# Lightbrite88/Argon_Monte_Carlo

Measured on AMD Instinct MI355X. Metric: particle-steps/sec, higher is better.
Workload: dtype f64; 1 GPU; cube_1e5; geometry=cube, n_particles=100000, n_per_gpu=100000, parallelism=single GPU

## Files before the change

argon_monte_carlo_amd/csrc/amc_commit_dev.h:

```cpp
#pragma once
#include "amc_grid_dev.h"

#define AMC_COMMIT_BLOCKS 64

struct amc_commit_args {
    amc_resolve_ctl *ctl;
    const double4 *hist;
    int *ov_head;
    const int *ev_gen;
    const rs_event *ev;
    const int4 *sl_meta;
    const int *sl_hits;
    const uint8_t *sl_moved;
    const double *sl_state;
    int *slot_of;
    int max_slots, max_hist;
    long long lo, hi;
    int count_pp;
    int defer;
    int nogrid;
    int enabled;
    int step;
    const int *od_stall;
    int od_tick;
    int from_wide;
    const int *wctl;
    int *host_ncand;
};

AMC_DEV void amc_commit_part(const amc_commit_args &C, const amc_out &O, const amc_grid &G, const amc_state &S, int gtid,
                             int gstride)
{
    amc_resolve_ctl *ctl = C.ctl;
    int c_active, c_ok, c_nslots, c_nhist, c_ncand, c_nclusters = 0, c_rounds;
    if (C.from_wide) {
        const amc_resolve_ctl *wc = (const amc_resolve_ctl *)C.wctl;
        c_ncand = wc->ncand;
        c_active = c_ncand > 0;
        c_nslots = 2 * c_ncand + wc->nslots; c_nhist = 4 * c_ncand + wc->nhist;
        c_ok = !wc->ovf; c_rounds = 1;
        if (gtid == 0) {
            for (int b = 0; b < 16; b++) c_nclusters += C.wctl[32 + b];
            if (C.host_ncand) *C.host_ncand = c_ncand;
            O.cnt->cand_count = 0;
        }
    } else {
        c_active = ctl->active; c_ok = ctl->ok && !ctl->ovf; c_nslots = ctl->nslots; c_nhist = ctl->nhist;
        c_ncand = ctl->ncand; c_rounds = ctl->rounds;
        if (gtid == 0) c_nclusters = ctl->nclusters;
    }
    if (!c_active) return;
    const bool ok = c_ok != 0;
    const bool defer = ok && C.defer;
    const int ns = c_nslots < C.max_slots ? c_nslots : C.max_slots;
    const int nh = c_nhist < C.max_hist ? c_nhist : C.max_hist;
    int my_hits = 0, my_fp = 0;
    for (int s = gtid; s < ns; s += gstride) {
        const int p = C.sl_meta[s].x;
        if (ok && C.count_pp) { const int hs = C.sl_hits[s]; my_hits += hs & 0xffff; my_fp += hs >> 16; }
        if (defer || p < 0) continue;
        if (ok && C.sl_moved[s]) {
            const double *t = C.sl_state + (size_t)s * RS_SLOT_DOUBLES;
            S.x[p] = t[0]; S.y[p] = t[1]; S.z[p] = t[2]; S.vx[p] = t[3]; S.vy[p] = t[4]; S.vz[p] = t[5];
            S.d[p] = t[6]; S.dx[p] = t[7]; S.dy[p] = t[8]; S.dz[p] = t[9]; S.flag[p] = t[10] != 0.0 ? 1 : 0;
        }
        C.slot_of[p] = -1;
    }
    for (int o = 32; o > 0; o >>= 1) { my_hits += __shfl_down(my_hits, o, 64); my_fp += __shfl_down(my_fp, o, 64); }
    if ((threadIdx.x & 63) == 0 && my_hits) atomicAdd(&O.banks[amc_bank_id()].n_pp, (unsigned long long)my_hits);
    if ((threadIdx.x & 63) == 0 && my_fp) atomicAdd(&O.banks[amc_bank_id()].n_fp_errors, (unsigned long long)my_fp);
    if (ok)
        for (int e = gtid; e < nh; e += gstride) {
            const int g = C.ev_gen[e];
            if (g == 0) continue;
            const rs_event ev = C.ev[e];
            if (g != C.sl_meta[ev.slot].z) continue;
            const int owner = ev.which ? ev.i : ev.j;
            if (owner < C.lo || owner >= C.hi) continue;
            amc_emit(O, ev.phase, ev.cell, ev.i, ev.j, ev.which, ev.val[0], ev.val[1], ev.val[2], ev.val[3]);
        }
    if (!C.nogrid)
        for (int h = gtid; h < nh; h += gstride) {
            const double4 r = C.hist[h];
            int cx, cy, cz;
            amc_grid_coords(G, r.x, r.y, r.z, cx, cy, cz);
            C.ov_head[amc_grid_cell(G, cx, cy, cz, nullptr)] = -1;
        }
    if (gtid == 0) {
        amc_dev_counters *cnt = O.cnt;
        cnt->n_candidates += (unsigned long long)c_ncand;
        cnt->n_clusters += (unsigned long long)c_nclusters;
        cnt->n_rounds += (unsigned long long)c_rounds;
        if (!ok) cnt->flags |= 4ULL;
        ctl->lazy_ns = defer ? ns : 0;
    }
}
```

argon_monte_carlo_amd/csrc/amc_grid.hip:

```cpp
#include <stdlib.h>

#include "amc_grid_dev.h"

#define AMC_CR2_INFLATE (1.0 + 1.0e-9)

__global__ __launch_bounds__(256) void k_bin_lists(const double *__restrict__ x, const double *__restrict__ y,
                                                   const double *__restrict__ z, long long n, amc_grid G, amc_lists B,
                                                   amc_dev_counters *cnt, amc_ovl V)
{
    const long long p = (long long)blockIdx.x * blockDim.x + threadIdx.x;
    if (p >= n) return;
    if (V.skip_epoch && (unsigned int)(V.adj_head[p] >> 32) == V.skip_epoch) return;
    bool outside = false;
    amc_list_insert(G, B, (int)p, x[p], y[p], z[p], &outside);
    if (outside) atomicOr(&cnt->flags, 8ULL);
}

struct amc_adj {
    unsigned long long *head;
    int4 *rec;
    int4 *sd;
    int4 *sl_meta;
    int *sl_hits, *ev_gen;
    unsigned int epoch;
    unsigned long long *mark;
};

AMC_DEV int amc_push_candidate(int a, int b, int max_cand, amc_dev_counters *cnt, const amc_adj &D)
{
    const unsigned int k = atomicAdd(&cnt->cand_count, 1u);
    if (k < (unsigned)max_cand) {
        const int hi = a > b ? a : b, lo = a > b ? b : a;
        int4 r;
        r.x = hi; r.y = lo; r.z = -1; r.w = -1;
        if (D.head) {
            const unsigned long long mine = ((unsigned long long)D.epoch << 32) | (unsigned long long)k;
            const unsigned long long oi = atomicExch(&D.head[hi], mine), oj = atomicExch(&D.head[lo], mine);
            r.z = ((unsigned int)(oi >> 32) == D.epoch) ? (int)(unsigned int)(oi & 0xffffffffULL) : -1;
            r.w = ((unsigned int)(oj >> 32) == D.epoch) ? (int)(unsigned int)(oj & 0xffffffffULL) : -1;
            auto mark = [&](int kd) {
                const unsigned long long old = atomicExch(&D.mark[kd], mine);
                if ((unsigned int)(old >> 32) == D.epoch) D.mark[kd] = ((unsigned long long)D.epoch << 32) | AMC_MARK_MULTI;
            };
            if (r.z >= 0) mark(r.z);
            if (r.w >= 0) mark(r.w);
        }
        D.rec[k] = r;
        D.sd[k] = make_int4(-1, -1, 0, 0);
        if (D.head) {
            D.sl_meta[2 * k] = make_int4(-1, 2 * (int)k, 0, 0);
            D.sl_meta[2 * k + 1] = make_int4(-1, 2 * (int)k + 1, 0, 0);
            atomicAnd(&D.sl_hits[2 * k], 0);
            atomicAnd(&D.sl_hits[2 * k + 1], 0);
            *(int4 *)&D.ev_gen[4 * k] = make_int4(0, 0, 0, 0);
        }
        return (int)k;
    }
    atomicOr(&cnt->flags, 1ULL);
    return -1;
}

AMC_DEV void amc_detect_node(const amc_grid &G, const amc_lists &B, int node, double cr2i, double cr_probe, int max_cand,
                             amc_dev_counters *cnt, const amc_adj &D, const int *od_stall = nullptr, int od_tick = 0)
{
    const int stalled = od_stall ? *od_stall : 0;
    amc_rec me_r = B.rec[node];
    const int live = (B.node_of && node < B.n) ? B.node_of[node] : node;
    if (stalled && od_tick > stalled) return;
    if (me_r.x != me_r.x) {
        if (live == node) return;
        node = live;
        me_r = B.rec[node];
        if (me_r.x != me_r.x) return;
    }
    const int me_p = amc_node_particle(B, node);
    double3 me;
    amc_rec_pos(G, me_r, me.x, me.y, me.z);
    auto found_pair = [&](int q) { amc_push_candidate(me_p, amc_node_particle(B, q), max_cand, cnt, D); };
    int q[9];
    q[0] = amc_rec_next(me_r);
    {
        int ocx, ocy, ocz;
        amc_grid_coords(G, me.x, me.y, me.z, ocx, ocy, ocz);
        const int c_own = amc_grid_cell(G, ocx, ocy, ocz, nullptr);
        int c_lo[4], c_hi[4];
        const int nc = amc_grid_box_ranges(G, me.x, me.y, me.z, cr_probe, c_lo, c_hi);
        int cell[8];
#pragma unroll
        for (int k = 0; k < 4; k++)
#pragma unroll
            for (int t = 0; t < 2; t++) {
                const int c = c_lo[k < nc ? k : 0] + t;
                cell[2 * k + t] = (k < nc && c <= c_hi[k < nc ? k : 0] && c < c_own) ? c : -1;
            }
        unsigned long long hv[8];
#pragma unroll
        for (int e = 0; e < 8; e++) hv[e] = (cell[e] >= 0) ? B.head[cell[e]] : 0ULL;
#pragma unroll
        for (int e = 0; e < 8; e++)
            q[1 + e] = (cell[e] >= 0 && (unsigned int)(hv[e] >> 32) == B.epoch) ? (int)(unsigned int)(hv[e] & 0xffffffffULL) : -1;
    }
    for (;;) {
        bool live = false;
#pragma unroll
        for (int e = 0; e < 9; e++) live |= q[e] >= 0;
        if (!live) break;
        amc_rec o[9];
#pragma unroll
        for (int e = 0; e < 9; e++)
            if (q[e] >= 0) o[e] = B.rec[q[e]];
#pragma unroll
        for (int e = 0; e < 9; e++)
            if (q[e] >= 0) {
                double ox, oy, oz;
                amc_rec_pos(G, o[e], ox, oy, oz);
                const double ex = ox - me.x, ey = oy - me.y, ez = oz - me.z;
                if (ex * ex + ey * ey + ez * ez < cr2i) found_pair(q[e]);
                q[e] = amc_rec_next(o[e]);
            }
    }
}

#ifndef AMC_DETECT_MINW
#define AMC_DETECT_MINW 4
#endif
__global__ __launch_bounds__(256, AMC_DETECT_MINW) void k_detect_lists(amc_grid G, amc_lists B, long long n, double cr2i, double cr_probe,
                                                      int max_cand, amc_dev_counters *cnt, amc_adj D, const int *extra_count,
                                                      int max_extra, const int *od_stall, int od_tick, int *wctl_rearm)
{
    const long long nb = (n + blockDim.x - 1) / blockDim.x;
    if ((long long)blockIdx.x < nb) {
        const long long p = (long long)blockIdx.x * blockDim.x + threadIdx.x;
        if (p < n) amc_detect_node(G, B, (int)p, cr2i, cr_probe, max_cand, cnt, D, od_stall, od_tick);
        if (wctl_rearm && p == 0 && !(*od_stall && od_tick > *od_stall)) {
            amc_resolve_ctl *wc = (amc_resolve_ctl *)wctl_rearm;
            for (int b = 0; b < 16; b++) wctl_rearm[32 + b] = 0;
            wc->nslots = 0; wc->nhist = 0; wc->nedges = 0; wc->nfp = 0; wc->ovf = 0; wc->dirty = 0; wc->nclusters = 0;
            wc->changed = 0; wc->active = 0; wc->cur_round = 1;
        }
        return;
    }
    if (!extra_count) return;
    int ne = *extra_count;
    if (ne > max_extra) ne = max_extra;
    const int stride = (int)((gridDim.x - nb) * blockDim.x);
    for (int e = (int)((blockIdx.x - nb) * blockDim.x + threadIdx.x); e < ne; e += stride)
        amc_detect_node(G, B, (int)n + e, cr2i, cr_probe, max_cand, cnt, D, od_stall, od_tick);
}

__global__ __launch_bounds__(256) void k_detect_own(amc_grid G, amc_lists B, long long lo, long long hi, double cr2i,
                                                    double cr_probe, int *__restrict__ out, int cap, amc_dev_counters *cnt)
{
    const long long p = lo + (long long)blockIdx.x * blockDim.x + threadIdx.x;
    if (p >= hi) return;
    amc_rec me_r = B.rec[p];
    const int live = B.node_of ? B.node_of[p] : (int)p;
    if (me_r.x != me_r.x) {
        if (live == (int)p) return;
        me_r = B.rec[live];
        if (me_r.x != me_r.x) return;
    }
    double3 me;
    amc_rec_pos(G, me_r, me.x, me.y, me.z);
    int c_lo[4], c_hi[4];
    const int nc = amc_grid_box_ranges(G, me.x, me.y, me.z, cr_probe, c_lo, c_hi);
    int q[8];
    unsigned long long hv[8];
#pragma unroll
    for (int k = 0; k < 4; k++)
#pragma unroll
        for (int t = 0; t < 2; t++) {
            const int c = c_lo[k < nc ? k : 0] + t;
            const bool on = k < nc && c <= c_hi[k < nc ? k : 0];
            hv[2 * k + t] = on ? B.head[c] : 0ULL;
            q[2 * k + t] = on ? 0 : -1;
        }
#pragma unroll
    for (int e = 0; e < 8; e++)
        q[e] = (q[e] == 0 && (unsigned int)(hv[e] >> 32) == B.epoch) ? (int)(unsigned int)(hv[e] & 0xffffffffULL) : -1;
    for (;;) {
        bool live = false;
#pragma unroll
        for (int e = 0; e < 8; e++) live |= q[e] >= 0;
        if (!live) break;
        amc_rec o[8];
#pragma unroll
        for (int e = 0; e < 8; e++)
            if (q[e] >= 0) o[e] = B.rec[q[e]];
#pragma unroll
        for (int e = 0; e < 8; e++)
            if (q[e] >= 0) {
                double ox, oy, oz;
                amc_rec_pos(G, o[e], ox, oy, oz);
                const double ex = ox - me.x, ey = oy - me.y, ez = oz - me.z;
                const int pq = amc_node_particle(B, q[e]);
                if (pq < (int)p && ex * ex + ey * ey + ez * ez < cr2i) {
                    const int k = atomicAdd(&out[0], 1);
                    if (k < cap) { out[2 + 2 * k] = (int)p; out[3 + 2 * k] = pq; }
                    else atomicOr(&cnt->flags, 1ULL);
                }
                q[e] = amc_rec_next(o[e]);
            }
    }
}

__global__ __launch_bounds__(256) void k_ingest_candidates(const int *__restrict__ blocks, int world, int block_ints, int cap,
                                                           int max_cand, amc_dev_counters *cnt, amc_adj D, int *__restrict__ own)
{
    const int gtid = blockIdx.x * blockDim.x + threadIdx.x, gstride = gridDim.x * blockDim.x;
    for (int r = 0; r < world; r++) {
        const int *b = blocks + (size_t)r * block_ints;
        int nr = b[0];
        if (nr > cap) {
            nr = cap;
            if (gtid == 0) atomicOr(&cnt->flags, 1ULL);
        }
        for (int k = gtid; k < nr; k += gstride) amc_push_candidate(b[2 + 2 * k], b[3 + 2 * k], max_cand, cnt, D);
    }
    if (gtid == 0) own[0] = 0;
}

#define AP_T 256
__global__ __launch_bounds__(AP_T) void k_detect_allpairs(const double *__restrict__ x, const double *__restrict__ y,
                                                          const double *__restrict__ z, int n, int ntiles, double cr2i,
                                                          int max_cand, amc_dev_counters *cnt, amc_adj D)
{
    int bi = (int)((sqrt(8.0 * (double)blockIdx.x + 1.0) - 1.0) * 0.5);
    while ((long long)(bi + 1) * (bi + 2) / 2 <= (long long)blockIdx.x) bi++;
    while ((long long)bi * (bi + 1) / 2 > (long long)blockIdx.x) bi--;
    const int bj = (int)(blockIdx.x - (long long)bi * (bi + 1) / 2);
    if (bi >= ntiles) return;
    __shared__ double tx[AP_T], ty[AP_T], tz[AP_T];
    const int j0 = bj * AP_T;
    const int jj = j0 + threadIdx.x;
    tx[threadIdx.x] = (jj < n) ? x[jj] : 0.0;
    ty[threadIdx.x] = (jj < n) ? y[jj] : 0.0;
    tz[threadIdx.x] = (jj < n) ? z[jj] : 0.0;
    __syncthreads();
    const int i = bi * AP_T + threadIdx.x;
    if (i >= n) return;
    const double xi = x[i], yi = y[i], zi = z[i];
    int jmax = n - j0;
    if (jmax > AP_T) jmax = AP_T;
    if (bi == bj && jmax > (int)threadIdx.x) jmax = threadIdx.x;
#pragma unroll 4
    for (int k = 0; k < jmax; k++) {
        const double ex = tx[k] - xi, ey = ty[k] - yi, ez = tz[k] - zi;
        const double d2 = fma(ez, ez, fma(ey, ey, ex * ex));
        if (d2 < cr2i) amc_push_candidate(i, j0 + k, max_cand, cnt, D);
    }
}

hipError_t amc_launch_bin(amc_ctx *c)
{
    if (c->allpairs || c->n <= 0) return hipSuccess;
    const long long n = c->n;
    c->B.epoch++;
    c->step.lists_age = -1;
    amc_prof_begin(c, AMC_K_BIN_COUNT);
    amc_ovl V;
    V.adj_head = nullptr; V.skip_epoch = 0;
    AMC_LAUNCH(c, k_bin_lists, dim3((unsigned)((n + 255) / 256)), dim3(256), c->S.x, c->S.y, c->S.z, n,
                       c->G, c->B, c->d_cnt, V);
    amc_prof_end(c);
    return hipGetLastError();
}

hipError_t amc_launch_bin_ovl(amc_ctx *c, int to, unsigned int skip_epoch, hipStream_t stream)
{
    const long long n = c->n;
    amc_ovl V;
    V.adj_head = c->W.adj_head; V.skip_epoch = skip_epoch;
    amc_prof_begin(c, AMC_K_BIN_COUNT);
    AMC_LAUNCH_ON(c, stream, k_bin_lists, dim3((unsigned)((n + 255) / 256)), dim3(256), c->S_buf[to].x, c->S_buf[to].y, c->S_buf[to].z, n,
                  c->G, c->B_buf[to], c->d_cnt, V);
    amc_prof_end(c);
    return hipGetLastError();
}

#define AP2_T 1024
#define AP2_R 4
#define AP2_THREADS (AP2_T / AP2_R)
#define AP2_CHUNK 8
__global__ __launch_bounds__(AP2_THREADS) void k_detect_allpairs_tiled(const double *__restrict__ x, const double *__restrict__ y,
                                                               const double *__restrict__ z, int n, int ntiles, double thr,
                                                               double ox, double oy, double oz,
                                                               int max_cand, amc_dev_counters *cnt, amc_adj D)
{
    int bi = (int)((sqrt(8.0 * (double)blockIdx.x + 1.0) - 1.0) * 0.5);
    while ((long long)(bi + 1) * (bi + 2) / 2 <= (long long)blockIdx.x) bi++;
    while ((long long)bi * (bi + 1) / 2 > (long long)blockIdx.x) bi--;
    const int bj = (int)(blockIdx.x - (long long)bi * (bi + 1) / 2);
    if (bi >= ntiles) return;
    __shared__ double tx[AP2_T], ty[AP2_T], tz[AP2_T], tn[AP2_T];
    const int j0 = bj * AP2_T;
    for (int t = threadIdx.x; t < AP2_T; t += AP2_THREADS) {
        const int jj = j0 + t;
        const bool in = jj < n;
        const double X = in ? x[jj] - ox : 0.0, Y = in ? y[jj] - oy : 0.0, Z = in ? z[jj] - oz : 0.0;
        tx[t] = X; ty[t] = Y; tz[t] = Z;
        tn[t] = in ? fma(Z, Z, fma(Y, Y, X * X)) : 1.0e300;
    }
    __syncthreads();
    int ii[AP2_R];
    double ax[AP2_R], ay[AP2_R], az[AP2_R], ti[AP2_R];
#pragma unroll
    for (int r = 0; r < AP2_R; r++) {
        ii[r] = bi * AP2_T + r * AP2_THREADS + (int)threadIdx.x;
        const bool in = ii[r] < n;
        const double X = in ? x[ii[r]] - ox : 0.0, Y = in ? y[ii[r]] - oy : 0.0, Z = in ? z[ii[r]] - oz : 0.0;
        ax[r] = -2.0 * X; ay[r] = -2.0 * Y; az[r] = -2.0 * Z;
        ti[r] = in ? thr - fma(Z, Z, fma(Y, Y, X * X)) : -1.0e300;
    }
    const bool diag = bi == bj;
    for (int k0 = 0; k0 < AP2_T; k0 += AP2_CHUNK) {
        bool any = false;
#pragma unroll
        for (int u = 0; u < AP2_CHUNK; u++) {
            const double jx = tx[k0 + u], jy = ty[k0 + u], jz = tz[k0 + u], jn = tn[k0 + u];
#pragma unroll
            for (int r = 0; r < AP2_R; r++) any |= fma(az[r], jz, fma(ay[r], jy, fma(ax[r], jx, jn))) < ti[r];
        }
        if (any) {
            for (int u = 0; u < AP2_CHUNK; u++) {
                const int j = j0 + k0 + u;
                const double jx = tx[k0 + u], jy = ty[k0 + u], jz = tz[k0 + u], jn = tn[k0 + u];
#pragma unroll
                for (int r = 0; r < AP2_R; r++)
                    if (fma(az[r], jz, fma(ay[r], jy, fma(ax[r], jx, jn))) < ti[r] && (diag ? j < ii[r] : true))
                        amc_push_candidate(ii[r], j, max_cand, cnt, D);
            }
        }
    }
}

static unsigned int next_sweep_epoch(unsigned int epoch)
{
    epoch = (epoch + 1u) & 0x3fffffffu;
    return epoch ? epoch : 1u;
}

hipError_t amc_launch_detect(amc_ctx *c)
{
    const long long n = c->n;
    if (n <= 0) return hipSuccess;
    const double cr2i = c->allpairs || c->detect_ap ? c->P.collision_range * c->P.collision_range * AMC_CR2_INFLATE : c->G.cr2_probe;
    amc_adj D;
    c->step.sweep_epoch = next_sweep_epoch(c->step.sweep_epoch);
    c->step.plan_split = !c->allpairs && !(c->h_host_ncand && *c->h_host_ncand <= c->plan_small);
    D.head = c->allpairs ? nullptr : c->W.adj_head; D.rec = c->W.cand4; D.sd = c->W.cand_s; D.epoch = c->step.sweep_epoch;
    D.sl_meta = c->W.sl_meta; D.sl_hits = c->W.sl_hits; D.ev_gen = c->W.ev_gen; D.mark = c->W.cand_mark;
    amc_prof_begin(c, AMC_K_DETECT);
    if (c->detect_ap) {
        if (n >= 16 * AP2_T && c->G.ncells > 0) {
            const int ntiles = (int)((n + AP2_T - 1) / AP2_T);
            const long long nblocks = (long long)ntiles * (ntiles + 1) / 2;
            const double ex = c->G.gx * c->G.h, ey = c->G.gy * c->G.h, ez = c->G.gz * c->G.h;
            const double thr = cr2i + 64.0 * 1.1102230246251565e-16 * (ex * ex + ey * ey + ez * ez);
            AMC_LAUNCH(c, k_detect_allpairs_tiled, dim3((unsigned)nblocks), dim3(AP2_THREADS), c->S.x, c->S.y,
                               c->S.z, (int)n, ntiles, thr, c->G.x0, c->G.y0, c->G.z0, c->W.max_cand, c->d_cnt, D);
        } else {
            const int ntiles = (int)((n + AP_T - 1) / AP_T);
            const long long nblocks = (long long)ntiles * (ntiles + 1) / 2;
            if (nblocks > 0)
                AMC_LAUNCH(c, k_detect_allpairs, dim3((unsigned)nblocks), dim3(AP_T), c->S.x, c->S.y,
                                   c->S.z, (int)n, ntiles, cr2i, c->W.max_cand, c->d_cnt, D);
        }
    } else {
        const bool extras = c->B.extra != nullptr && c->keep_K < 2;
        const int slot = (c->B.extra == c->extra_buf[1]) ? 1 : 0;
        const int bs = c->detect_bs;
        AMC_LAUNCH(c, k_detect_lists, dim3((unsigned)((n + bs - 1) / bs) + (extras ? 4u : 0u)), dim3(bs), c->G, c->B, n, cr2i,
                   c->G.cr_probe, c->W.max_cand, c->d_cnt, D, (const int *)(extras ? c->extra_count + slot : nullptr),
                   c->max_extra, (const int *)(c->od_active ? c->d_od : nullptr), c->od_tick,
                   (c->od_active && !c->step.od_prev_ordered) ? c->W.wctl : nullptr);
    }
    amc_prof_end(c);
    return hipGetLastError();
}

hipError_t amc_launch_detect_own(amc_ctx *c)
{
    const long long cnt = c->hi - c->lo;
    amc_prof_begin(c, AMC_K_DETECT);
    if (cnt > 0)
        AMC_LAUNCH(c, k_detect_own, dim3((unsigned)((cnt + 255) / 256)), dim3(256), c->G, c->B, (long long)c->lo, (long long)c->hi,
                   c->G.cr2_probe, c->G.cr_probe, c->MG.cand_send, c->MG.cand_cap, c->d_cnt);
    amc_prof_end(c);
    return hipGetLastError();
}

hipError_t amc_launch_ingest(amc_ctx *c, int world)
{
    amc_adj D;
    c->step.sweep_epoch = next_sweep_epoch(c->step.sweep_epoch);
    c->step.plan_split = !(c->h_host_ncand && *c->h_host_ncand <= c->plan_small);
    D.head = c->W.adj_head; D.rec = c->W.cand4; D.sd = c->W.cand_s; D.epoch = c->step.sweep_epoch;
    D.sl_meta = c->W.sl_meta; D.sl_hits = c->W.sl_hits; D.ev_gen = c->W.ev_gen; D.mark = c->W.cand_mark;
    amc_prof_begin(c, AMC_K_DETECT);
    AMC_LAUNCH(c, k_ingest_candidates, dim3(16), dim3(256), (const int *)c->MG.cand_recv, world, 2 + 2 * c->MG.cand_cap, c->MG.cand_cap,
               c->W.max_cand, c->d_cnt, D, c->MG.cand_send);
    amc_prof_end(c);
    return hipGetLastError();
}
```

argon_monte_carlo_amd/csrc/amc_stream.hip:

```cpp
#include <stdlib.h>
#include <string.h>

#include <algorithm>

#include "amc_commit_dev.h"
#include "amc_energised_dev.h"

struct amc_stream_counts {
    int nwall, nerr, noob, noob_pre;
};

template <int GEOM>
AMC_DEV void amc_stream_particle(amc_particle &q, const amc_params &P, const amc_out &O, double dt, int stages, int ip,
                                 double &px, double &py, double &pz, amc_stream_counts &cn)
{
    if ((stages & AMC_ST_BOUNDS_PRE) && GEOM != AMC_GEOM_CUBE)
        cn.noob_pre = amc_bounds(P, q.x, q.y, q.z, GEOM == AMC_GEOM_PORE_ENERGISED);
    if (stages & AMC_ST_DRIFT) {
        px = q.x; py = q.y; pz = q.z;
        const double sx = dt * q.vx, sy = dt * q.vy, sz = dt * q.vz;
        q.x += sx; q.y += sy; q.z += sz;
        q.d += fabs(sqrt(sx * sx + sy * sy + sz * sz));
        q.dx += fabs(sx); q.dy += fabs(sy); q.dz += fabs(sz);
    }
    if (stages & AMC_ST_WALLS) {
        if (GEOM == AMC_GEOM_CUBE) {
#define AMC_CUBE_AXIS(pos, vel, W)                                                                    \
    if (pos > W) { const double t_ = (pos - W) / vel; vel = -vel; pos = W + t_ * vel; }                \
    if (pos < 0) { const double t_ = pos / vel; vel = -vel; pos = t_ * vel; }
            AMC_CUBE_AXIS(q.x, q.vx, P.cube_x)
            AMC_CUBE_AXIS(q.y, q.vy, P.cube_y)
            AMC_CUBE_AXIS(q.z, q.vz, P.cube_z)
#undef AMC_CUBE_AXIS
        } else if (GEOM == AMC_GEOM_PORE) {
            const double zb = P.z_gap_bottom, zt = P.z_gap_top;
            const double r0 = sqrt(px * px + py * py);
            if (sqrt(q.x * q.x + q.y * q.y) > P.R_oa) {
                if (amc_side_wall(q, P.R_oa_c, true, O, 1, ip)) cn.nerr++; else cn.nwall++;
            }
            if (q.z < 0) { amc_vertical_wall(q, 0.0, O, 2, ip); cn.nwall++; }
            if (q.z > P.H) { amc_vertical_wall(q, P.H, O, 3, ip); cn.nwall++; }
            if ((pz > P.z_cold) && (q.z < P.z_cold) && (sqrt(q.x * q.x + q.y * q.y) > P.R_p)) {
                amc_vertical_wall(q, P.z_cold, O, 4, ip); cn.nwall++;
            }
            if ((pz < P.h_oa) && (q.z > P.h_oa) && (sqrt(q.x * q.x + q.y * q.y) > P.R_p)) {
                amc_vertical_wall(q, P.h_oa, O, 5, ip); cn.nwall++;
            }
            if ((pz < zt) && (pz > zb) && (r0 < P.R_g) && (sqrt(q.x * q.x + q.y * q.y) > P.R_g)) {
                if (amc_side_wall(q, P.R_g_c, true, O, 6, ip)) cn.nerr++; else cn.nwall++;
            }
            if ((r0 > P.R_p) && (q.z < zb) && (pz < zt) && (pz > zb)) {
                amc_vertical_wall(q, zb, O, 7, ip); cn.nwall++;
            }
            if ((r0 > P.R_p) && (q.z > zt) && (pz < zt) && (pz > zb)) {
                amc_vertical_wall(q, zt, O, 8, ip); cn.nwall++;
            }
            if ((r0 < P.R_p) && (sqrt(q.x * q.x + q.y * q.y) > P.R_p) &&
                (((q.z < P.z_cold) && (q.z > zt)) || ((q.z < zb) && (q.z > P.h_oa)))) {
                if (amc_side_wall(q, P.R_p_c, true, O, 9, ip)) cn.nerr++; else cn.nwall++;
            }
        } else if (GEOM == AMC_GEOM_PORE_ENERGISED) {
            if (sqrt(q.x * q.x + q.y * q.y) > P.R_oa) {
                if (amc_side_wall(q, P.R_oa_c, false, O, 1, ip)) cn.nerr++;
            }
            if (q.z < 0) { const double t_ = (q.z - 0.0) / q.vz; q.vz = -q.vz; q.z = 0.0 + t_ * q.vz; }
            if (q.z > P.H) { const double t_ = (q.z - P.H) / q.vz; q.vz = -q.vz; q.z = P.H + t_ * q.vz; }
        }
    }
    if ((stages & AMC_ST_BOUNDS) && GEOM != AMC_GEOM_CUBE)
        cn.noob = amc_bounds(P, q.x, q.y, q.z, GEOM == AMC_GEOM_PORE_ENERGISED);
}

AMC_DEV void amc_stream_count(const amc_out &O, const amc_stream_counts &cn, int bounds_slot, int ip)
{
    if (!(cn.nwall | cn.nerr | cn.noob | cn.noob_pre)) return;
    if (O.wev.count) {
        amc_wev_rec r;
        r.p = ip; r.kind = 1; r.a = cn.nwall | (cn.nerr << 16); r.b = cn.noob | (cn.noob_pre << 16);
        r.v[0] = r.v[1] = r.v[2] = r.v[3] = 0.0;
        amc_wev_append(O, r);
        return;
    }
    if (cn.nwall) atomicAdd(&O.banks[amc_bank_id()].n_wall, (unsigned long long)cn.nwall);
    if (cn.nerr) atomicAdd(&O.banks[amc_bank_id()].n_fp_errors, (unsigned long long)cn.nerr);
    if (cn.noob) atomicAdd(bounds_slot ? &O.cnt->n_oob_pp : &O.cnt->n_oob_walls, (unsigned long long)cn.noob);
    if (cn.noob_pre) atomicAdd(&O.cnt->n_oob_pp, (unsigned long long)cn.noob_pre);
}

#define AMC_LD(p) __builtin_nontemporal_load(&(p))
#define AMC_ST(p, v) __builtin_nontemporal_store((v), &(p))

template <int GEOM, int TEMP = 0>
__global__ __launch_bounds__(256) void k_stream(amc_state S, amc_state S_out, amc_params P, amc_out O, double dt, int stages,
                                                long long lo, long long hi, int keep_prior, int bounds_slot,
                                                amc_grid G, amc_lists B, int build_lists, amc_lazy L, amc_commit_args C,
                                                amc_ovl V, const amc_temp_pass *TP)
{
    const int stalled = C.od_stall ? *C.od_stall : 0;
    if (C.enabled) {
        const unsigned nstream = gridDim.x - (unsigned)C.enabled;
        if (blockIdx.x >= nstream) {
            if (stalled && C.od_tick > stalled) return;
            amc_out Oc = O;
            Oc.step = C.step;
            amc_commit_part(C, Oc, G, S, (int)((blockIdx.x - nstream) * blockDim.x + threadIdx.x), (int)(C.enabled * blockDim.x));
            return;
        }
    }
    const long long p = lo + (long long)blockIdx.x * blockDim.x + threadIdx.x;
    if (p >= hi) return;
    if (V.skip_epoch && (unsigned int)(V.adj_head[p] >> 32) == V.skip_epoch) return;
    const int wave_id = (int)(blockIdx.x * (blockDim.x >> 6) + (threadIdx.x >> 6));
    const int keep_count0 = build_lists == 3 ? B.wave_count[wave_id] : 0;
    const int keep_cell = build_lists == 3 ? B.cell_of[p] : -1, keep_node = build_lists == 3 ? B.node_of[p] : (int)p;
    amc_particle q;
    q.x = AMC_LD(S.x[p]); q.y = AMC_LD(S.y[p]); q.z = AMC_LD(S.z[p]);
    q.vx = AMC_LD(S.vx[p]); q.vy = AMC_LD(S.vy[p]); q.vz = AMC_LD(S.vz[p]);
    const double x_in = q.x, y_in = q.y, z_in = q.z, vx_in = q.vx, vy_in = q.vy, vz_in = q.vz;
    const bool need_acc = (stages & (AMC_ST_DRIFT | AMC_ST_WALLS)) != 0;
    bool flag_in = false;
    double d_in = 0, dx_in = 0, dy_in = 0, dz_in = 0;
    q.d = q.dx = q.dy = q.dz = 0; q.flag = false;
    if (need_acc) {
        q.d = AMC_LD(S.d[p]); q.dx = AMC_LD(S.dx[p]); q.dy = AMC_LD(S.dy[p]); q.dz = AMC_LD(S.dz[p]);
        q.flag = S.flag[p] != 0;
        flag_in = q.flag; d_in = q.d; dx_in = q.dx; dy_in = q.dy; dz_in = q.dz;
    }
    if (stalled && C.od_tick > stalled) return;
    bool force = S_out.x != S.x;
    if (L.enabled) {
        const int sl = L.slot_of[p];
        if (sl >= 0) {
            L.slot_of[p] = -1;
            if (L.moved[sl]) {
                const double *t = L.state + (size_t)sl * RS_SLOT_DOUBLES;
                q.x = t[0]; q.y = t[1]; q.z = t[2]; q.vx = t[3]; q.vy = t[4]; q.vz = t[5];
                q.d = t[6]; q.dx = t[7]; q.dy = t[8]; q.dz = t[9]; q.flag = t[10] != 0.0;
                force = true;
            }
        }
    }
    const bool wr_acc = need_acc || force;
    double px = q.x, py = q.y, pz = q.z;
    if (!(stages & AMC_ST_DRIFT) && GEOM != AMC_GEOM_CUBE && (stages & AMC_ST_WALLS)) { px = S.px[p]; py = S.py[p]; pz = S.pz[p]; }
    amc_stream_counts cn = {0, 0, 0, 0};
    const bool temp_cases = GEOM == AMC_GEOM_PORE_ENERGISED && TEMP != 0;
    amc_stream_particle<GEOM>(q, P, O, dt, temp_cases ? (stages & ~AMC_ST_BOUNDS) : stages, (int)p, px, py, pz, cn);
    if ((stages & AMC_ST_DRIFT) && keep_prior && GEOM != AMC_GEOM_CUBE) { S.px[p] = px; S.py[p] = py; S.pz[p] = pz; }
    if (GEOM == AMC_GEOM_PORE_ENERGISED && TEMP != 0) {
        if (temp_any_mask(P, q.x, q.y, q.z, px, py, pz)) {
            temp_particle t;
            t.x = q.x; t.y = q.y; t.z = q.z; t.vx = q.vx; t.vy = q.vy; t.vz = q.vz;
            t.d = q.d; t.dx = q.dx; t.dy = q.dy; t.dz = q.dz; t.flag = q.flag ? 1 : 0; t.nwall = 0; t.nerr = 0;
            temp_cases_particle<true>(P, O, TP->g, (unsigned int)O.step, TP->D, (int)p, px, py, pz, t);
            q.x = t.x; q.y = t.y; q.z = t.z; q.vx = t.vx; q.vy = t.vy; q.vz = t.vz;
            q.d = t.d; q.dx = t.dx; q.dy = t.dy; q.dz = t.dz; q.flag = t.flag != 0;
            cn.nwall += t.nwall; cn.nerr += t.nerr;
        }
        if (stages & AMC_ST_BOUNDS) cn.noob = amc_bounds(P, q.x, q.y, q.z, true);
    }

    if (force || q.x != x_in) AMC_ST(S_out.x[p], q.x);
    if (force || q.y != y_in) AMC_ST(S_out.y[p], q.y);
    if (force || q.z != z_in) AMC_ST(S_out.z[p], q.z);
    if (force || q.vx != vx_in) S_out.vx[p] = q.vx;
    if (force || q.vy != vy_in) S_out.vy[p] = q.vy;
    if (force || q.vz != vz_in) S_out.vz[p] = q.vz;
    if (wr_acc) {
        if (force || q.d != d_in) AMC_ST(S_out.d[p], q.d);
        if (force || q.dx != dx_in) AMC_ST(S_out.dx[p], q.dx);
        if (force || q.dy != dy_in) AMC_ST(S_out.dy[p], q.dy);
        if (force || q.dz != dz_in) AMC_ST(S_out.dz[p], q.dz);
        if (force || q.flag != flag_in) S_out.flag[p] = q.flag ? 1 : 0;
    }
    if (build_lists == 1) {
        bool outside = false;
        amc_list_insert(G, B, (int)p, q.x, q.y, q.z, &outside);
        if (outside) atomicOr(&O.cnt->flags, 8ULL);
    } else if (build_lists) {
        bool outside = false, overflow = false;
        const int nc = amc_list_keep(G, B, (int)p, q.x, q.y, q.z, build_lists == 2, wave_id, keep_count0, keep_cell, keep_node, &outside, &overflow);
        if ((int)__lane_id() == __ffsll((long long)__ballot(true)) - 1) B.wave_count[wave_id] = nc;
        if (outside) atomicOr(&O.cnt->flags, 8ULL);
        if (overflow) atomicOr(&O.cnt->flags, 1ULL);
    }
    amc_stream_count(O, cn, bounds_slot, (int)p);
}

struct amc_fixup_args {
    amc_state S_in, S_out;
    amc_lists B;
    int *extra;
    int *extra_count;
    int max_extra;
    const unsigned long long *adj_head;
    const unsigned int *victim;
    unsigned int sweep_epoch;
    amc_wev wev;
    unsigned int *wev_clear;
    int *extra_clear;
    int stages, step_sweep, step_stream;
    double dt;
};

#define AMC_FIXUP_SLOT_BLOCKS 24

template <int GEOM>
__global__ __launch_bounds__(256) void k_fixup(amc_fixup_args F, amc_params P, amc_out O, amc_grid G, amc_commit_args C)
{
    if (blockIdx.x == 0 && threadIdx.x < AMC_COUNTER_BANKS) F.wev_clear[threadIdx.x] = 0;
    if (blockIdx.x == 0 && threadIdx.x == 0) *F.extra_clear = 0;
    if (F.sweep_epoch && blockIdx.x < AMC_FIXUP_SLOT_BLOCKS) {
        const int gtid = blockIdx.x * blockDim.x + threadIdx.x, gstride = AMC_FIXUP_SLOT_BLOCKS * blockDim.x;
        amc_resolve_ctl *ctl = C.ctl;
        const bool active = ctl->active != 0;
        const bool ok = ctl->ok && !ctl->ovf;
        const int ns = !active ? 0 : (ctl->nslots < C.max_slots ? ctl->nslots : C.max_slots);
        amc_out Od = O;
        Od.wev.count = nullptr;
        Od.step = F.step_stream;
        for (int s = gtid; s < ns; s += gstride) {
            const int p = C.sl_meta[s].x;
            if (p < 0) continue;
            amc_particle q;
            if (ok && C.sl_moved[s]) {
                const double *t = C.sl_state + (size_t)s * RS_SLOT_DOUBLES;
                q.x = t[0]; q.y = t[1]; q.z = t[2]; q.vx = t[3]; q.vy = t[4]; q.vz = t[5];
                q.d = t[6]; q.dx = t[7]; q.dy = t[8]; q.dz = t[9]; q.flag = t[10] != 0.0;
            } else {
                q.x = F.S_in.x[p]; q.y = F.S_in.y[p]; q.z = F.S_in.z[p]; q.vx = F.S_in.vx[p]; q.vy = F.S_in.vy[p]; q.vz = F.S_in.vz[p];
                q.d = F.S_in.d[p]; q.dx = F.S_in.dx[p]; q.dy = F.S_in.dy[p]; q.dz = F.S_in.dz[p]; q.flag = F.S_in.flag[p] != 0;
            }
            const bool marked = (unsigned int)(F.adj_head[p] >> 32) == F.sweep_epoch;
            double px = q.x, py = q.y, pz = q.z;
            amc_stream_counts cn = {0, 0, 0, 0};
            amc_stream_particle<GEOM>(q, P, Od, F.dt, F.stages, p, px, py, pz, cn);
            F.S_out.x[p] = q.x; F.S_out.y[p] = q.y; F.S_out.z[p] = q.z;
            F.S_out.vx[p] = q.vx; F.S_out.vy[p] = q.vy; F.S_out.vz[p] = q.vz;
            F.S_out.d[p] = q.d; F.S_out.dx[p] = q.dx; F.S_out.dy[p] = q.dy; F.S_out.dz[p] = q.dz; F.S_out.flag[p] = q.flag ? 1 : 0;
            bool outside = false;
            if (marked) {
                amc_list_insert(G, F.B, p, q.x, q.y, q.z, &outside);
            } else {
                ((float *)&F.B.rec[p])[0] = __int_as_float(0x7fc00000);
                const int e = atomicAdd(F.extra_count, 1);
                atomicAdd(&O.cnt->n_refiled, 1);
                if (e < F.max_extra) {
                    F.extra[e] = p;
                    amc_list_insert(G, F.B, F.B.n + e, q.x, q.y, q.z, &outside);
                } else {
                    atomicOr(&O.cnt->flags, 4ULL);
                }
            }
            if (outside) atomicOr(&O.cnt->flags, 8ULL);
            C.slot_of[p] = -1;
            amc_stream_count(Od, cn, 0, p);
        }
    } else if (F.sweep_epoch) {
        amc_out Os = O;
        Os.wev.count = nullptr;
        Os.step = F.step_sweep;
        amc_commit_part(C, Os, G, F.S_in, (int)((blockIdx.x - AMC_FIXUP_SLOT_BLOCKS) * blockDim.x + threadIdx.x),
                        (int)((gridDim.x - AMC_FIXUP_SLOT_BLOCKS) * blockDim.x));
    }
    amc_out Od = O;
    Od.wev.count = nullptr;
    Od.step = F.step_stream;
    for (int b = blockIdx.x; b < AMC_COUNTER_BANKS; b += gridDim.x) {
        unsigned int nb = F.wev.count[b];
        if (nb > (unsigned)F.wev.cap) nb = (unsigned)F.wev.cap;
        for (unsigned int k = threadIdx.x; k < nb; k += blockDim.x) {
            const amc_wev_rec r = F.wev.rec[(size_t)b * F.wev.cap + k];
            if (F.sweep_epoch && F.victim[r.p] == F.sweep_epoch) continue;
            if (r.kind == 0) {
                amc_emit(Od, r.a, 0, r.p, -1, 0, r.v[0], r.v[1], r.v[2], r.v[3]);
            } else {
                amc_stream_counts cn = {r.a & 0xffff, r.a >> 16, r.b & 0xffff, r.b >> 16};
                amc_stream_count(Od, cn, 0, r.p);
            }
        }
    }
}

amc_commit_args amc_make_commit_args(amc_ctx *c)
{
    const amc_resolve_ws &W = c->W;
    amc_commit_args C;
    C.ctl = (amc_resolve_ctl *)W.ctl; C.hist = W.hist; C.ov_head = W.ov_head; C.ev_gen = W.ev_gen; C.ev = W.ev;
    C.sl_meta = W.sl_meta; C.sl_hits = W.sl_hits; C.sl_moved = W.sl_moved; C.sl_state = W.sl_state; C.slot_of = W.slot_of;
    C.max_slots = W.max_slots; C.max_hist = W.max_hist; C.lo = c->lo; C.hi = c->hi; C.count_pp = c->MG.count_pp ? 1 : 0;
    C.defer = c->step.commit_defer ? 1 : 0; C.nogrid = c->allpairs ? 1 : 0; C.enabled = 0;
    C.step = c->step.commit_step;
    C.od_stall = nullptr; C.od_tick = 0; C.from_wide = 0; C.wctl = nullptr; C.host_ncand = nullptr;
    return C;
}

int amc_list_build_mode(amc_ctx *c, int owner, bool kept)
{
    amc_step_state &T = c->step;
    if (!kept) { c->B.epoch++; T.lists_age = -1; return 1; }
    if (T.lists_owner != owner) T.lists_age = -1;
    T.lists_owner = owner;
    if (T.lists_age < 0 || T.lists_age + 1 >= c->keep_K) { c->B.epoch++; T.lists_age = 0; T.full_builds++; return 2; }
    T.lists_age++;
    return 3;
}

static void launch_k_stream(amc_ctx *c, hipStream_t stream, unsigned blocks, int threads, const amc_state &S, const amc_state &S_out,
                            const amc_out &O, double dt, int stages, long long lo, long long hi, int keep_prior, int bounds_slot,
                            const amc_lists &B, int build, const amc_lazy &L, const amc_commit_args &C, const amc_ovl &V)
{
    const bool cases = (stages & AMC_ST_TEMP_CASES) != 0;
    auto *k = k_stream<AMC_GEOM_CUBE>;
    switch (c->P.geometry) {
    case AMC_GEOM_CUBE: break;
    case AMC_GEOM_PORE: k = k_stream<AMC_GEOM_PORE>; break;
    case AMC_GEOM_PORE_ENERGISED: k = cases ? k_stream<AMC_GEOM_PORE_ENERGISED, 1> : k_stream<AMC_GEOM_PORE_ENERGISED>; break;
    default: return;
    }
    AMC_LAUNCH_ON(c, stream, k, dim3(blocks), dim3(threads), S, S_out, c->P, O, dt, stages, lo, hi, keep_prior, bounds_slot, c->G, B,
                  build, L, C, V, (const amc_temp_pass *)(cases ? c->TD.pass : nullptr));
}

hipError_t amc_launch_stream(amc_ctx *c, double dt, int stages, int bounds_slot, bool fuse_bin)
{
    const int threads = c->stream_bs;
    int build = 0;
    if (fuse_bin && !c->allpairs && c->lo == 0 && c->hi == c->n) build = amc_list_build_mode(c, 1, c->keep_K >= 2 && c->B.cell_of);
    amc_lazy L;
    memset(&L, 0, sizeof L);
    if (c->step.lazy_pending) {
        const amc_resolve_ws &W = c->W;
        L.slot_of = W.slot_of; L.state = W.sl_state; L.moved = W.sl_moved;
        L.enabled = 1;
        c->step.lazy_pending = false;
    }
    const long long cnt = c->hi - c->lo;
    if (cnt <= 0) return hipSuccess;
    amc_commit_args C = amc_make_commit_args(c);
    const amc_resolve_ws &W_ = c->W;
    unsigned extra = 0;
    if (c->step.commit_pending) {
        const long long lag = c->h_host_ncand ? *c->h_host_ncand : 0;
        extra = (unsigned)std::min<long long>(std::max<long long>((2 * lag + 255) / 256, 4), AMC_COMMIT_BLOCKS);
        C.enabled = (int)extra;
        c->step.commit_pending = false;
        if (c->od_active && !c->step.od_prev_ordered) { C.from_wide = 1; C.wctl = W_.wctl; C.host_ncand = c->d_host_ncand; }
    }
    if (c->od_active) { C.od_stall = c->d_od; C.od_tick = c->od_tick; }
    const unsigned blocks = (unsigned)((cnt + threads - 1) / threads) + extra;
    const int kp = (stages & AMC_ST_TEMP_CASES) ? (int)(c->P.reserved0 & 1) : (c->keep_prior ? 1 : 0);
    amc_ovl V;
    V.adj_head = nullptr; V.skip_epoch = 0;
    if ((stages & AMC_ST_TEMP_CASES) && (c->P.geometry != AMC_GEOM_PORE_ENERGISED || !c->TD.pass)) return hipErrorInvalidValue;
    amc_prof_begin(c, (stages == AMC_ST_BOUNDS) ? AMC_K_BOUNDS : AMC_K_DRIFT_WALLS);
    launch_k_stream(c, c->stream, blocks, threads, c->S, c->S, c->out, dt, stages, c->lo, c->hi, kp, bounds_slot, c->B, build, L, C, V);
    amc_prof_end(c);
    return hipGetLastError();
}

hipError_t amc_launch_stream_ovl(amc_ctx *c, double dt, int stages, int from, unsigned int skip_epoch, hipStream_t stream,
                                 bool build_lists)
{
    const int to = 1 - from;
    amc_lists &Bn = c->B_buf[to];
    Bn.epoch++;
    c->step.lists_age = -1;
    amc_lazy L;
    memset(&L, 0, sizeof L);
    amc_commit_args C = amc_make_commit_args(c);
    amc_ovl V;
    V.adj_head = c->W.adj_head; V.skip_epoch = skip_epoch;
    amc_out O = c->out;
    O.wev = c->wev_buf[c->out.step & 1];
    const unsigned blocks = (unsigned)((c->n + 255) / 256);
    amc_prof_begin(c, AMC_K_DRIFT_WALLS);
    launch_k_stream(c, stream, blocks, 256, c->S_buf[from], c->S_buf[to], O, dt, stages, 0, c->n, 0, 0, Bn, build_lists ? 1 : 0, L, C, V);
    amc_prof_end(c);
    return hipGetLastError();
}

hipError_t amc_launch_fixup(amc_ctx *c, double dt, int stages, int from, unsigned int sweep_epoch)
{
    const int to = 1 - from;
    amc_fixup_args F;
    F.S_in = c->S_buf[from]; F.S_out = c->S_buf[to];
    F.B = c->B_buf[to];
    F.extra = c->extra_buf[to]; F.extra_count = c->extra_count + to; F.max_extra = c->max_extra;
    F.adj_head = c->W.adj_head; F.victim = c->W.victim; F.sweep_epoch = sweep_epoch;
    F.wev = c->wev_buf[c->out.step & 1];
    F.wev_clear = c->wev_buf[1 - (c->out.step & 1)].count;
    F.extra_clear = c->extra_count + from;
    F.stages = stages; F.step_stream = c->out.step; F.step_sweep = c->out.step - 1; F.dt = dt;
    amc_commit_args C = amc_make_commit_args(c);
    C.defer = 1;
    C.enabled = 1;
    amc_prof_begin(c, AMC_K_FIXUP);
    if (c->P.geometry == AMC_GEOM_CUBE)
        AMC_LAUNCH(c, k_fixup<AMC_GEOM_CUBE>, dim3(AMC_COMMIT_BLOCKS), dim3(256), F, c->P, c->out, c->G, C);
    else
        AMC_LAUNCH(c, k_fixup<AMC_GEOM_PORE>, dim3(AMC_COMMIT_BLOCKS), dim3(256), F, c->P, c->out, c->G, C);
    amc_prof_end(c);
    return hipGetLastError();
}
```

Baseline: 2.349 billion particle-steps/s.

## Issue commit and detect loads early to hide global-memory latency

Splits the commit pass into an 'ask' phase that speculatively loads the first slot, event and history entries plus the control words, then an 'apply' phase that uses them, so these loads are in flight before the stall check. The per-block cluster-count sum becomes a wave shuffle reduction instead of a serial loop on thread 0. The detect kernel reorders its arguments, passes precomputed block count and size, and moves the stall load after the record load so the loads overlap. Counter updates become atomics, which adds a little cost but makes them safe under concurrency.

```diff
diff --git a/argon_monte_carlo_amd/csrc/amc_commit_dev.h b/argon_monte_carlo_amd/csrc/amc_commit_dev.h
--- a/argon_monte_carlo_amd/csrc/amc_commit_dev.h
+++ b/argon_monte_carlo_amd/csrc/amc_commit_dev.h
@@ -28,70 +28,107 @@
     int *host_ncand;
 };
 
-AMC_DEV void amc_commit_part(const amc_commit_args &C, const amc_out &O, const amc_grid &G, const amc_state &S, int gtid,
-                             int gstride)
+struct amc_commit_first {
+    int active, ok, nslots, nhist, ncand, nclusters, rounds;
+    int4 meta;
+    int hits;
+    int gen;
+    rs_event ev;
+    double4 h;
+};
+
+AMC_DEV void amc_commit_ask(const amc_commit_args &C, int gtid, amc_commit_first &F)
+{
+    const int is = gtid < C.max_slots ? gtid : 0, ih = gtid < C.max_hist ? gtid : 0;
+    F.meta = C.sl_meta[is]; F.hits = C.sl_hits[is];
+    F.gen = C.ev_gen[ih]; F.ev = C.ev[ih]; F.h = C.hist[ih];
+    if (C.from_wide) {
+        const amc_resolve_ctl *wc = (const amc_resolve_ctl *)C.wctl;
+        const int w_ncand = wc->ncand, w_nslots = wc->nslots, w_nhist = wc->nhist, w_ovf = wc->ovf;
+        const int nc = C.wctl[32 + (threadIdx.x & 15)];
+        F.ncand = w_ncand; F.active = w_ncand > 0;
+        F.nslots = 2 * w_ncand + w_nslots; F.nhist = 4 * w_ncand + w_nhist;
+        F.ok = w_ovf == 0; F.rounds = 1; F.nclusters = nc;
+    } else {
+        const amc_resolve_ctl *ctl = C.ctl;
+        const int c_active = ctl->active, c_ok = ctl->ok, c_ovf = ctl->ovf;
+        F.nslots = ctl->nslots; F.nhist = ctl->nhist; F.ncand = ctl->ncand; F.rounds = ctl->rounds; F.nclusters = ctl->nclusters;
+        F.active = c_active; F.ok = (c_ok != 0) & (c_ovf == 0);
+    }
+    asm volatile("" ::: "memory");
+}
+
+AMC_DEV void amc_commit_apply(const amc_commit_args &C, const amc_out &O, const amc_grid &G, const amc_state &S, int gtid,
+                              int gstride, const amc_commit_first &F)
 {
     amc_resolve_ctl *ctl = C.ctl;
-    int c_active, c_ok, c_nslots, c_nhist, c_ncand, c_nclusters = 0, c_rounds;
-    if (C.from_wide) {
-        const amc_resolve_ctl *wc = (const amc_resolve_ctl *)C.wctl;
-        c_ncand = wc->ncand;
-        c_active = c_ncand > 0;
-        c_nslots = 2 * c_ncand + wc->nslots; c_nhist = 4 * c_ncand + wc->nhist;
-        c_ok = !wc->ovf; c_rounds = 1;
-        if (gtid == 0) {
-            for (int b = 0; b < 16; b++) c_nclusters += C.wctl[32 + b];
-            if (C.host_ncand) *C.host_ncand = c_ncand;
-            O.cnt->cand_count = 0;
-        }
-    } else {
-        c_active = ctl->active; c_ok = ctl->ok && !ctl->ovf; c_nslots = ctl->nslots; c_nhist = ctl->nhist;
-        c_ncand = ctl->ncand; c_rounds = ctl->rounds;
-        if (gtid == 0) c_nclusters = ctl->nclusters;
+    const int c_active = F.active, c_ok = F.ok, c_nslots = F.nslots, c_nhist = F.nhist, c_ncand = F.ncand, c_rounds = F.rounds;
+    int c_nclusters = F.nclusters;
+    if (C.from_wide)
+        for (int o = 8; o > 0; o >>= 1) c_nclusters += __shfl_xor(c_nclusters, o, 64);
+    if (C.from_wide && gtid == 0) {
+        if (C.host_ncand) *C.host_ncand = c_ncand;
+        O.cnt->cand_count = 0;
     }
     if (!c_active) return;
     const bool ok = c_ok != 0;
     const bool defer = ok && C.defer;
+    const bool count = ok && C.count_pp;
     const int ns = c_nslots < C.max_slots ? c_nslots : C.max_slots;
     const int nh = c_nhist < C.max_hist ? c_nhist : C.max_hist;
     int my_hits = 0, my_fp = 0;
-    for (int s = gtid; s < ns; s += gstride) {
-        const int p = C.sl_meta[s].x;
-        if (ok && C.count_pp) { const int hs = C.sl_hits[s]; my_hits += hs & 0xffff; my_fp += hs >> 16; }
-        if (defer || p < 0) continue;
+    auto slot = [&](int s, int p, int hs) {
+        my_hits += hs & 0xffff; my_fp += hs >> 16;
+        if (defer || p < 0) return;
         if (ok && C.sl_moved[s]) {
             const double *t = C.sl_state + (size_t)s * RS_SLOT_DOUBLES;
             S.x[p] = t[0]; S.y[p] = t[1]; S.z[p] = t[2]; S.vx[p] = t[3]; S.vy[p] = t[4]; S.vz[p] = t[5];
             S.d[p] = t[6]; S.dx[p] = t[7]; S.dy[p] = t[8]; S.dz[p] = t[9]; S.flag[p] = t[10] != 0.0 ? 1 : 0;
         }
         C.slot_of[p] = -1;
-    }
+    };
+    if (gtid < ns) slot(gtid, F.meta.x, count ? F.hits : 0);
+    for (int s = gtid + gstride; s < ns; s += gstride) slot(s, C.sl_meta[s].x, count ? C.sl_hits[s] : 0);
     for (int o = 32; o > 0; o >>= 1) { my_hits += __shfl_down(my_hits, o, 64); my_fp += __shfl_down(my_fp, o, 64); }
     if ((threadIdx.x & 63) == 0 && my_hits) atomicAdd(&O.banks[amc_bank_id()].n_pp, (unsigned long long)my_hits);
     if ((threadIdx.x & 63) == 0 && my_fp) atomicAdd(&O.banks[amc_bank_id()].n_fp_errors, (unsigned long long)my_fp);
-    if (ok)
-        for (int e = gtid; e < nh; e += gstride) {
+    auto event = [&](int g, const rs_event &ev) {
+        if (g != C.sl_meta[(unsigned)ev.slot].z) return;
+        const int owner = ev.which ? ev.i : ev.j;
+        if (owner < C.lo || owner >= C.hi) return;
+        amc_emit(O, ev.phase, ev.cell, ev.i, ev.j, ev.which, ev.val[0], ev.val[1], ev.val[2], ev.val[3]);
+    };
+    if (ok) {
+        if (gtid < nh && F.gen != 0) event(F.gen, F.ev);
+        for (int e = gtid + gstride; e < nh; e += gstride) {
             const int g = C.ev_gen[e];
             if (g == 0) continue;
-            const rs_event ev = C.ev[e];
-            if (g != C.sl_meta[ev.slot].z) continue;
-            const int owner = ev.which ? ev.i : ev.j;
-            if (owner < C.lo || owner >= C.hi) continue;
-            amc_emit(O, ev.phase, ev.cell, ev.i, ev.j, ev.which, ev.val[0], ev.val[1], ev.val[2], ev.val[3]);
+            event(g, C.ev[e]);
         }
-    if (!C.nogrid)
-        for (int h = gtid; h < nh; h += gstride) {
-            const double4 r = C.hist[h];
+    }
+    if (!C.nogrid) {
+        auto clear = [&](const double4 &r) {
             int cx, cy, cz;
             amc_grid_coords(G, r.x, r.y, r.z, cx, cy, cz);
             C.ov_head[amc_grid_cell(G, cx, cy, cz, nullptr)] = -1;
-        }
+        };
+        if (gtid < nh) clear(F.h);
+        for (int h = gtid + gstride; h < nh; h += gstride) clear(C.hist[h]);
+    }
     if (gtid == 0) {
         amc_dev_counters *cnt = O.cnt;
-        cnt->n_candidates += (unsigned long long)c_ncand;
-        cnt->n_clusters += (unsigned long long)c_nclusters;
-        cnt->n_rounds += (unsigned long long)c_rounds;
-        if (!ok) cnt->flags |= 4ULL;
+        atomicAdd(&cnt->n_candidates, (unsigned long long)c_ncand);
+        atomicAdd(&cnt->n_clusters, (unsigned long long)c_nclusters);
+        atomicAdd(&cnt->n_rounds, (unsigned long long)c_rounds);
+        if (!ok) atomicOr(&cnt->flags, 4ULL);
         ctl->lazy_ns = defer ? ns : 0;
     }
 }
+
+AMC_DEV void amc_commit_part(const amc_commit_args &C, const amc_out &O, const amc_grid &G, const amc_state &S, int gtid,
+                             int gstride)
+{
+    amc_commit_first F;
+    amc_commit_ask(C, gtid, F);
+    amc_commit_apply(C, O, G, S, gtid, gstride, F);
+}
diff --git a/argon_monte_carlo_amd/csrc/amc_grid.hip b/argon_monte_carlo_amd/csrc/amc_grid.hip
--- a/argon_monte_carlo_amd/csrc/amc_grid.hip
+++ b/argon_monte_carlo_amd/csrc/amc_grid.hip
@@ -63,9 +63,9 @@
 AMC_DEV void amc_detect_node(const amc_grid &G, const amc_lists &B, int node, double cr2i, double cr_probe, int max_cand,
                              amc_dev_counters *cnt, const amc_adj &D, const int *od_stall = nullptr, int od_tick = 0)
 {
-    const int stalled = od_stall ? *od_stall : 0;
     amc_rec me_r = B.rec[node];
     const int live = (B.node_of && node < B.n) ? B.node_of[node] : node;
+    const int stalled = od_stall ? *od_stall : 0;
     if (stalled && od_tick > stalled) return;
     if (me_r.x != me_r.x) {
         if (live == node) return;
@@ -124,13 +124,14 @@
 #ifndef AMC_DETECT_MINW
 #define AMC_DETECT_MINW 4
 #endif
-__global__ __launch_bounds__(256, AMC_DETECT_MINW) void k_detect_lists(amc_grid G, amc_lists B, long long n, double cr2i, double cr_probe,
+__global__ __launch_bounds__(256, AMC_DETECT_MINW) void k_detect_lists(amc_rec *rec, const int *od_stall, long long n, int od_tick,
+                                                      int nb, int bs, amc_grid G, amc_lists B, double cr2i, double cr_probe,
                                                       int max_cand, amc_dev_counters *cnt, amc_adj D, const int *extra_count,
-                                                      int max_extra, const int *od_stall, int od_tick, int *wctl_rearm)
-{
-    const long long nb = (n + blockDim.x - 1) / blockDim.x;
-    if ((long long)blockIdx.x < nb) {
-        const long long p = (long long)blockIdx.x * blockDim.x + threadIdx.x;
+                                                      int max_extra, int *wctl_rearm)
+{
+    B.rec = rec;
+    if ((int)blockIdx.x < nb) {
+        const long long p = (long long)blockIdx.x * bs + threadIdx.x;
         if (p < n) amc_detect_node(G, B, (int)p, cr2i, cr_probe, max_cand, cnt, D, od_stall, od_tick);
         if (wctl_rearm && p == 0 && !(*od_stall && od_tick > *od_stall)) {
             amc_resolve_ctl *wc = (amc_resolve_ctl *)wctl_rearm;
@@ -143,8 +144,8 @@
     if (!extra_count) return;
     int ne = *extra_count;
     if (ne > max_extra) ne = max_extra;
-    const int stride = (int)((gridDim.x - nb) * blockDim.x);
-    for (int e = (int)((blockIdx.x - nb) * blockDim.x + threadIdx.x); e < ne; e += stride)
+    const int stride = (int)((gridDim.x - nb) * bs);
+    for (int e = (int)((blockIdx.x - nb) * bs + threadIdx.x); e < ne; e += stride)
         amc_detect_node(G, B, (int)n + e, cr2i, cr_probe, max_cand, cnt, D, od_stall, od_tick);
 }
 
@@ -370,10 +371,11 @@
         const bool extras = c->B.extra != nullptr && c->keep_K < 2;
         const int slot = (c->B.extra == c->extra_buf[1]) ? 1 : 0;
         const int bs = c->detect_bs;
-        AMC_LAUNCH(c, k_detect_lists, dim3((unsigned)((n + bs - 1) / bs) + (extras ? 4u : 0u)), dim3(bs), c->G, c->B, n, cr2i,
+        const int nb = (int)((n + bs - 1) / bs);
+        AMC_LAUNCH(c, k_detect_lists, dim3((unsigned)nb + (extras ? 4u : 0u)), dim3(bs), c->B.rec,
+                   (const int *)(c->od_active ? c->d_od : nullptr), n, c->od_tick, nb, bs, c->G, c->B, cr2i,
                    c->G.cr_probe, c->W.max_cand, c->d_cnt, D, (const int *)(extras ? c->extra_count + slot : nullptr),
-                   c->max_extra, (const int *)(c->od_active ? c->d_od : nullptr), c->od_tick,
-                   (c->od_active && !c->step.od_prev_ordered) ? c->W.wctl : nullptr);
+                   c->max_extra, (c->od_active && !c->step.od_prev_ordered) ? c->W.wctl : nullptr);
     }
     amc_prof_end(c);
     return hipGetLastError();
diff --git a/argon_monte_carlo_amd/csrc/amc_stream.hip b/argon_monte_carlo_amd/csrc/amc_stream.hip
--- a/argon_monte_carlo_amd/csrc/amc_stream.hip
+++ b/argon_monte_carlo_amd/csrc/amc_stream.hip
@@ -100,10 +100,13 @@
     if (C.enabled) {
         const unsigned nstream = gridDim.x - (unsigned)C.enabled;
         if (blockIdx.x >= nstream) {
+            const int ctid = (int)((blockIdx.x - nstream) * blockDim.x + threadIdx.x);
+            amc_commit_first F;
+            amc_commit_ask(C, ctid, F);
             if (stalled && C.od_tick > stalled) return;
             amc_out Oc = O;
             Oc.step = C.step;
-            amc_commit_part(C, Oc, G, S, (int)((blockIdx.x - nstream) * blockDim.x + threadIdx.x), (int)(C.enabled * blockDim.x));
+            amc_commit_apply(C, Oc, G, S, ctid, (int)(C.enabled * blockDim.x), F);
             return;
         }
     }
```

Measured after the change: 2.369 billion particle-steps/s, median of 6. About the same (+0.9%).
